# OpenGene/repaq

Hardware: AMD Instinct MI355X
Metric: raw FASTQ MB/s encode+decode (higher is better)
Workload: dtype u8; 1 GPU; configs[2]: synthetic NovaSeq PE150 two files (-i/-I), 2 x 4.01 GB FASTQ (fqgen profile 1, 11200000 pairs, seed 3, N 20 ppm), -k 1000, encode + decode; chunks_per_gpu=3360, parity=unchecked (checked with --full)

## Files before the change

### repaq_amd/csrc/enc/gather_tiles.h

```cpp
#pragma once
#define G2_CAP 23552u
#define G2_SE_OK 1
#define G2_CNT 256u
struct __attribute__((packed, aligned(1))) GU16g { uint32_t a, b, c, d; };
__device__ __forceinline__ void pack4_codes(uint32_t w, uint32_t& code, uint32_t& nb, uint32_t& bad) {
    const uint32_t idx = (w >> 1) & 0x03030303u;
    const uint32_t ok = eq_bytes_full(__builtin_amdgcn_perm(0u, 0x47544341u, idx), w);
    code = ((__builtin_amdgcn_perm(0u, 0x00020301u, idx) & ok) * 0x01041040u) >> 24;
    nb = 0; bad = 0;
    if (ok != 0xFFFFFFFFu) { const uint32_t isn = eq_bytes_full(w, 0x4E4E4E4Eu); nb = ((isn & 0x01010101u) * 0x01020408u) >> 24;
            bad = (((~ok & ~isn) & 0x01010101u) * 0x01020408u) >> 24; }
}
__device__ __forceinline__ void pack4_codes_rc(uint32_t w, uint32_t& code, uint32_t& nb) {
    const uint32_t u = w & 0xDFDFDFDFu, idx = (u >> 1) & 0x03030303u;
    const uint32_t ok = eq_bytes_full(__builtin_amdgcn_perm(0u, 0x47544341u, idx), u);
    code = ((__builtin_amdgcn_perm(0u, 0x03010002u, idx) & ok) * 0x01041040u) >> 24;
    nb = ((~ok & 0x01010101u) * 0x01020408u) >> 24;
}
__device__ __forceinline__ bool pack16_fast(const uint32_t (&w)[4], uint32_t& code) {
    uint32_t diff = 0; code = 0;
#pragma unroll
    for (int i = 0; i < 4; i++) {
        const uint32_t idx = (w[i] >> 1) & 0x03030303u;
        diff |= __builtin_amdgcn_perm(0u, 0x47544341u, idx) ^ w[i];
        code |= ((__builtin_amdgcn_perm(0u, 0x00020301u, idx) * 0x01041040u) >> 24) << (8 * i);
    }
    return diff == 0;
}
__device__ __forceinline__ uint32_t g2_rev2x16(uint32_t v) {
    v = bswap32(v); v = ((v >> 4) & 0x0F0F0F0Fu) | ((v & 0x0F0F0F0Fu) << 4); return ((v >> 2) & 0x33333333u) | ((v & 0x33333333u) << 2);
}
struct G2Geo { uint32_t a00, a01, end0, end1, base1; };
struct G2Read { bool on, rc; uint32_t len, qsrc, ssrc, qpos, ld, gi; };
struct G2Bound { uint32_t l0, l1, q; };
struct G2MRaw { uint4 lo4; uint32_t pg; };
#ifdef RFQ_SIMT_EMULATION
__device__ __forceinline__ uint32_t ld_uniform(const uint32_t* p) { return *p; }
#else
__device__ __forceinline__ uint32_t ld_uniform(const uint32_t* p) { return *(const __attribute__((address_space(4))) uint32_t*)(uintptr_t)p; }
#endif
__device__ __forceinline__ G2Bound g2_bound(const Text& T, bool two, const uint32_t* __restrict__ pq, uint32_t r) {
    G2Bound b;
    if (two) { const size_t k = 4 * (size_t)(r >> 1); b.l0 = ld_uniform(T.lo[0] + k); b.l1 = ld_uniform(T.lo[1] + k); }
    else { b.l0 = ld_uniform(T.lo[0] + 4 * (size_t)r); b.l1 = 0u; }
    b.q = ld_uniform(pq + r);
    return b;
}
__device__ __forceinline__ G2Geo g2_geo(const G2Bound& b, const G2Bound& e, bool two) {
    G2Geo g; g.a00 = b.l0 & ~15u; g.end0 = e.l0; g.a01 = two ? b.l1 & ~15u : 0u; g.end1 = two ? e.l1 : 0u;
    g.base1 = two ? (((g.end0 - g.a00 + 15u) & ~15u) + 16u) : 0u;
    return g;
}
__device__ __forceinline__ void g2_stage1(const uint8_t* __restrict__ fq, uint32_t n, uint32_t a0, uint32_t end, uint4* l4, uint32_t tid) {
    const uint32_t nb = end - a0, ng = (nb + 15u) / 16u;
    const uint8_t* src = fq + a0;
    const uint32_t nfull = (uint64_t)a0 + 16ull * ng <= (uint64_t)n ? ng : ng - 1u;
    for (uint32_t i = tid; i < nfull; i += blockDim.x)
        __builtin_amdgcn_global_load_lds((const __attribute__((address_space(1))) void*)(src + 16 * (size_t)i),
                (__attribute__((address_space(3))) void*)(l4 + (i - (tid & 63u))), 16, 0, 0);
    if (nfull < ng && tid == 0) { uint8_t* const bytes = (uint8_t*)l4;
            for (uint32_t k = 0; k < 16; k++) bytes[16 * nfull + k] = a0 + 16 * nfull + k < n ? src[16 * (size_t)nfull + k] : (uint8_t)0xFF; }
}
__device__ __forceinline__ void g2_stage(const Text& T, bool two, const G2Geo& g, uint4* buf4, uint32_t tid) {
    g2_stage1(T.fq[0], T.n[0], g.a00, g.end0, buf4, tid);
    if (two) g2_stage1(T.fq[1], T.n[1], g.a01, g.end1, buf4 + g.base1 / 16, tid);
}
__device__ __forceinline__ G2MRaw g2_mraw(const Text& T, const uint32_t* __restrict__ pq, uint32_t cur, uint32_t j, uint32_t cnt) {
    G2MRaw r; r.lo4 = make_uint4(0, 0, 0, 0); r.pg = 0;
    if (j < cnt) { const uint32_t gi = cur + j; int s_; uint32_t r_; read_loc(T, gi, s_, r_); r.lo4 = *(const uint4*)(t_lo(T, s_) + 4 * (size_t)r_); r.pg = pq[gi]; }
    return r;
}
__device__ __forceinline__ G2Read g2_read(const Text& T, const G2MRaw& r, const G2Geo& g, uint32_t f, uint32_t pq0, bool il, uint32_t cur, uint32_t j, uint32_t cnt) {
    G2Read m; m.on = j < cnt; m.rc = false; m.len = m.qsrc = m.ssrc = m.qpos = m.ld = 0; m.gi = cur + j;
    if (m.on) {
        const uint32_t gi = cur + j; int s_; uint32_t r_; read_loc(T, gi, s_, r_);
        const uint32_t lb = s_ ? g.base1 : 0u, a = s_ ? g.a01 : g.a00;
        m.len = r.lo4.z - 1u - r.lo4.y; m.ssrc = lb + (r.lo4.y - a); m.qsrc = lb + (r.lo4.w - a);
        m.qpos = r.pg - pq0; m.ld = (r.pg >> 4) + gi;
        m.rc = il && ((gi - f) & 1u);
    }
    return m;
}
__device__ __forceinline__ void g2_bases(const uint8_t* s_text, const G2Read& m, uint32_t part, uint32_t P, uint32_t* __restrict__ lpk, uint16_t* __restrict__ lnb,
        uint8_t* __restrict__ rflag, uint8_t* __restrict__ rn) {
    const uint32_t ng = (m.len + 15u) >> 4;
    for (uint32_t gi = part; gi < ng; gi += P) {
        uint32_t w[4], code = 0, nbits = 0;
        const uint32_t nv0 = m.len - 16u * gi;
        const bool tail = nv0 < 16u && m.len >= 16u; const uint32_t tsh = tail ? 16u - nv0 : 0u;
        auto blank = [&](uint32_t from, uint32_t to) { for (uint32_t k = from; k < to; k++) { uint32_t& x = w[k >> 2]; const uint32_t sh = 8u * (k & 3u);
                x = (x & ~(0xFFu << sh)) | (0x41u << sh); } };
        if (!m.rc) {
            lds_get16(s_text, m.ssrc + (tail ? m.len - 16u : 16u * gi), w);
            if (nv0 < 16u && !tail) blank(nv0, 16u);
            if (!pack16_fast(w, code)) {
                uint32_t bad = 0; code = 0;
#pragma unroll
                for (int i = 0; i < 4; i++) { uint32_t c4, n4, b4; pack4_codes(w[i], c4, n4, b4); code |= c4 << (8 * i); nbits |= n4 << (4 * i); bad |= b4 << (4 * i); }
                if (bad) rflag[m.gi] = 1;
            }
        } else {
            lds_get16(s_text, tail ? m.ssrc : m.ssrc + m.len - 16u * gi - 16u, w);
            if (nv0 < 16u && !tail) blank(0u, 16u - nv0);
            if (pack16_fast(w, code)) code = ~g2_rev2x16(code);
            else {
                const uint32_t x0 = bswap32(w[3]), x1 = bswap32(w[2]), x2 = bswap32(w[1]), x3 = bswap32(w[0]); w[0] = x0; w[1] = x1; w[2] = x2; w[3] = x3; code = 0;
#pragma unroll
                for (int i = 0; i < 4; i++) { uint32_t c4, n4; pack4_codes_rc(w[i], c4, n4); code |= c4 << (8 * i); nbits |= n4 << (4 * i); }
            }
        }
        code >>= 2u * tsh; nbits >>= tsh;
        if (nv0 < 16u) { code &= (1u << (2u * nv0)) - 1u; nbits &= (1u << nv0) - 1u; }
        lpk[m.ld + gi] = code; lnb[m.ld + gi] = (uint16_t)nbits;
        if (nbits) rn[m.gi] = 1;
    }
}
__device__ __forceinline__ void g2_compose(const uint8_t* s_text, const G2Read& m, uint32_t part, uint32_t P, uint8_t* qd, uint32_t* __restrict__ lpk,
        uint16_t* __restrict__ lnb, uint8_t* __restrict__ rflag, uint8_t* __restrict__ rn, QualCount& qc) {
    if (!m.on) return;
    {
        const uint32_t n = m.len; uint8_t* const o = qd + m.qpos; const bool rc = m.rc;
        if (n >= 16u) {
            const uint32_t ng = (n + 15u) >> 4;
            for (uint32_t gi = part; gi < ng; gi += P) {
                uint32_t p0 = 16u * gi, dup = 0; if (p0 + 16u > n) { dup = p0 + 16u - n; p0 = n - 16u; }
                uint32_t w[4]; lds_get16(s_text, rc ? m.qsrc + n - p0 - 16u : m.qsrc + p0, w);
                if (rc) { const uint32_t x0 = bswap32(w[3]), x1 = bswap32(w[2]), x2 = bswap32(w[1]), x3 = bswap32(w[0]); w[0] = x0; w[1] = x1; w[2] = x2; w[3] = x3; }
                { GU16g v; v.a = w[0]; v.b = w[1]; v.c = w[2]; v.d = w[3]; *(GU16g*)(o + p0) = v; }
                if (!dup) qc.group(m.qpos + p0, w[0], w[1], w[2], w[3]);
                else for (uint32_t k = dup; k < 16u; k++) qc(m.qpos + p0 + k, (uint8_t)(w[k >> 2] >> (8u * (k & 3u))));
            }
        } else for (uint32_t i = part; i < n; i += P) { const uint8_t q = s_text[rc ? m.qsrc + n - 1u - i : m.qsrc + i]; o[i] = q; qc(m.qpos + i, q); }
    }
    g2_bases(s_text, m, part, P, lpk, lnb, rflag, rn);
}
#define G2_REFN 256u
#define G2_REFS 128u
struct G2Ref { uint32_t nl, n1l, n2o, len, stl, lane, tile, nb, tb; int s; };
struct G2Acc { uint32_t bits, fail; };
__device__ __forceinline__ bool lane_bytes_eq(const uint8_t* tx, uint32_t a, uint32_t b, uint32_t n, bool on) {
    bool eq = true;
    for (uint32_t o = 0; __any(on && eq && o < n); o += 16u) {
        if (on && eq && o < n) {
            uint32_t p0 = o, v = n - o; if (v < 16u && n >= 16u) { p0 = n - 16u; v = 16u; }
            uint32_t x[4], y[4]; lds_get16(tx, a + p0, x); lds_get16(tx, b + p0, y);
            unsigned long long dl = (((unsigned long long)(x[1] ^ y[1])) << 32) | (x[0] ^ y[0]), dh = (((unsigned long long)(x[3] ^ y[3])) << 32) | (x[2] ^ y[2]);
            if (v < 16u) { dl &= v >= 8u ? ~0ull : (1ull << (8u * v)) - 1ull; dh &= v > 8u ? (1ull << (8u * (v - 8u))) - 1ull : 0ull; }
            if (dl | dh) eq = false;
        }
    }
    return eq;
}
__device__ __forceinline__ bool lane_bytes_eq32(const uint8_t* tx, uint32_t a, uint32_t b, uint32_t n) {
    uint32_t x[4], y[4]; lds_get16(tx, a, x); lds_get16(tx, b, y);
    unsigned long long dl = (((unsigned long long)(x[1] ^ y[1])) << 32) | (x[0] ^ y[0]), dh = (((unsigned long long)(x[3] ^ y[3])) << 32) | (x[2] ^ y[2]);
    if (n < 16u) { dl &= n >= 8u ? ~0ull : (1ull << (8u * n)) - 1ull; dh &= n > 8u ? (1ull << (8u * (n - 8u))) - 1ull : 0ull; }
    else { const uint32_t t = n - 16u; lds_get16(tx, a + t, x); lds_get16(tx, b + t, y); dl |= (((unsigned long long)(x[1] ^ y[1])) << 32) | (x[0] ^ y[0]);
            dh |= (((unsigned long long)(x[3] ^ y[3])) << 32) | (x[2] ^ y[2]); }
    return (dl | dh) == 0ull;
}
__device__ __forceinline__ bool g2_eq_ref(const uint8_t* tx, uint32_t a, uint32_t ro, uint32_t cap, const uint8_t* g0, uint32_t off0, uint32_t len0, uint32_t n,
        bool on) {
    const bool slow = on && len0 > cap, big = on && !slow && n > 32u; bool eq = true;
    if (on && !slow && !big && n) eq = lane_bytes_eq32(tx, a, ro + off0, n);
    if (__any(big)) { if (!lane_bytes_eq(tx, a, ro + off0, n, big)) eq = false; }
    if (slow) for (uint32_t i = 0; i < n && eq; i++) if (tx[a + i] != g0[off0 + i]) eq = false;
    return eq;
}
__device__ __forceinline__ uint32_t g2_atoi(const uint8_t* tx, uint32_t a, uint32_t n) {
    if (n == 0) return 0u;
    const unsigned long long w = lds_get8(tx, a); const uint32_t c0 = (uint32_t)w & 0xFFu;
    if (n > 8u || c0 == ' ' || (c0 >= 9u && c0 <= 13u) || c0 == '+' || c0 == '-') return (uint32_t)dev_atoi(tx + a, n);
    const unsigned long long x = w ^ 0x3030303030303030ull;
    const unsigned long long nd = (((x & 0x7F7F7F7F7F7F7F7Full) + 0x7676767676767676ull) | x) & 0x8080808080808080ull;
    uint32_t m = nd ? (uint32_t)(__ffsll((long long)nd) - 1) >> 3 : 8u; if (m > n) m = n;
    if (m == 0) return 0u;
    const unsigned long long X = x << (8u * (8u - m));
    const uint32_t hi4 = (uint32_t)X, lo4 = (uint32_t)(X >> 32);
    const uint32_t uh = ((hi4 << 3) + (hi4 << 1) + (hi4 >> 8)) & 0x00FF00FFu, ul = ((lo4 << 3) + (lo4 << 1) + (lo4 >> 8)) & 0x00FF00FFu;
    const uint32_t vh = mul24(uh & 0xFFu, 100u) + (uh >> 16), vl = mul24(ul & 0xFFu, 100u) + (ul >> 16);
    return mul24(vh, 10000u) + vl;
}
__device__ __forceinline__ uint32_t ctz64_or64(unsigned long long m) { return m ? (uint32_t)(__ffsll((long long)m) - 1) : 64u; }
__device__ __forceinline__ void g2_parse(const Text& T, const ReadTab& R, const uint8_t* tx, uint32_t refn, uint32_t refs, const G2Geo& g, const G2Ref& r0, uint32_t f,
        uint32_t cur, uint32_t cnt,
                                         bool can0, uint32_t dpos, uint32_t dch, G2Acc& acc) {
    const uint32_t l = (uint32_t)lane_id(); const bool on = l < cnt; const uint32_t gi = cur + l;
    uint32_t nsrc = 0, nl = 0, sl = 0, tsrc = 0, tl = 0;
    if (on) {
        int s_; uint32_t r_; read_loc(T, gi, s_, r_);
        const uint4 lo4 = *(const uint4*)(t_lo(T, s_) + 4 * (size_t)r_);
        const uint32_t lb = s_ ? g.base1 : 0u, a = s_ ? g.a01 : g.a00;
        nsrc = lb + (lo4.x - a); nl = lo4.y - 1u - lo4.x; sl = lo4.z - 1u - lo4.y; tsrc = lb + (lo4.z - a); tl = lo4.w - 1u - lo4.z;
    }
    unsigned long long Cm = 0, Sm = 0;
    {
        uint32_t c[4], sp_[4];
#pragma unroll
        for (int p = 0; p < 4; p++) { uint32_t w[4]; lds_get16(tx, nsrc + 16u * (uint32_t)p, w); const uint4 q = make_uint4(w[0], w[1], w[2], w[3]);
                c[p] = eq_mask16c(q, 0x3A3A3A3Au); sp_[p] = eq_mask16c(q, 0x20202020u); }
        const unsigned long long keep = !on ? 0ull : (nl >= 64u ? ~0ull : (1ull << nl) - 1ull);
        Cm = ((((unsigned long long)(c[2] | (c[3] << 16))) << 32) | (c[0] | (c[1] << 16))) & keep;
        Sm = ((((unsigned long long)(sp_[2] | (sp_[3] << 16))) << 32) | (sp_[0] | (sp_[1] << 16))) & keep;
    }
    const uint32_t sp = ctz64_or64(Sm);
    unsigned long long cb = sp < 64u ? Cm & ((1ull << sp) - 1ull) : Cm;
    const uint32_t k = (uint32_t)__popcll(cb);
    uint32_t cpos[8];
#pragma unroll
    for (int i = 1; i <= 7; i++) { cpos[i] = ctz64_or64(cb); cb &= cb - 1ull; }
    const bool at7 = cpos[7] < 64u, at_sp = !at7 && sp < 64u;
    const bool undecided = on && !at7 && !at_sp && nl > 64u;
    uint32_t ok = 0, n1l = nl, n2o = nl, lane_v = 0, tile_v = 0, x_v = 0, y_v = 0;
    if (on && (at7 || (at_sp && k >= 4u))) {
        ok = 1; n2o = at7 ? cpos[7] : sp;
        const bool k4 = at_sp && k == 4u, k5 = at_sp && k == 5u;
        n1l = k4 ? cpos[4] : cpos[3];
        const uint32_t ls = (k4 ? cpos[4] : cpos[3]) + 1u, le = k4 ? sp : cpos[4];
        lane_v = g2_atoi(tx, nsrc + ls, le - ls) & 0xFFu;
        if (k >= 5u) { const uint32_t ts = (k5 ? cpos[5] : cpos[4]) + 1u, te = k5 ? sp : cpos[5]; tile_v = g2_atoi(tx, nsrc + ts, te - ts) & 0xFFFFu; }
        if (k >= 6u) x_v = g2_atoi(tx, nsrc + cpos[5] + 1u, cpos[6] - cpos[5] - 1u);
        if (at7) y_v = g2_atoi(tx, nsrc + cpos[6] + 1u, cpos[7] - cpos[6] - 1u);
        else if (k == 6u) y_v = g2_atoi(tx, nsrc + cpos[6] + 1u, sp - cpos[6] - 1u);
    }
    if (__any(undecided)) {
        if (undecided) { const Meta m = dev_parse_name(tx + nsrc, nl); ok = m.ok; n1l = m.name1_len; n2o = m.name2_off; lane_v = m.lane; tile_v = m.tile; x_v = m.x;
                y_v = m.y; }
    }
    if (on) { R.name1_len[gi] = n1l; R.name2_off[gi] = n2o; R.x[gi] = x_v; R.y[gi] = y_v; R.tile[gi] = (uint16_t)tile_v; R.lane[gi] = (uint8_t)lane_v;
            R.ok[gi] = (uint8_t)ok; }
    const uint32_t n2l = nl - n2o, n2l0 = r0.nl - r0.n2o;
    const uint8_t* g0n = t_fq(T, r0.s) + r0.nb; const uint8_t* g0s = t_fq(T, r0.s) + r0.tb;
    const bool st_eq = g2_eq_ref(tx, tsrc, refs, G2_REFS, g0s, 0u, r0.stl, tl, on && tl == r0.stl);
    const bool n1_eq = g2_eq_ref(tx, nsrc, refn, G2_REFN, g0n, 0u, r0.nl, n1l, on && n1l == r0.n1l);
    const bool n2_eq = g2_eq_ref(tx, nsrc + n2o, refn, G2_REFN, g0n, r0.n2o, r0.nl, n2l, on && n2l == n2l0);
    const uint32_t pn = wave_shr1(nsrc, 0u), pnl = wave_shr1(nl, 0u), pn2o = wave_shr1(n2o, 0u), plane = wave_shr1(lane_v, 0u), ptile = wave_shr1(tile_v,
            0u), px = wave_shr1(x_v, 0u), py = wave_shr1(y_v, 0u);
    const uint32_t rel = gi - f; const bool odd = on && can0 && (rel & 1u);
    bool fa = false;
    if (__any(odd)) {
        const uint32_t pn2l = pnl - pn2o; const bool same_len = odd && pn2l == n2l;
        if (odd && !same_len) fa = true;
        const uint32_t ma = pn + pn2o, mb = nsrc + n2o; const bool small = same_len && n2l <= 16u, big = same_len && !small;
        if (small && n2l) {
            uint32_t x[4], y[4]; lds_get16(tx, ma, x); lds_get16(tx, mb, y);
            if (dch != 0u && dpos < n2l) {
                const uint32_t sh = 8u * (dpos & 3u);
#pragma unroll
                for (int q = 0; q < 4; q++) if ((dpos >> 2) == (uint32_t)q) x[q] = (x[q] & ~(0xFFu << sh)) | (dch << sh);
            }
            unsigned long long dl = (((unsigned long long)(x[1] ^ y[1])) << 32) | (x[0] ^ y[0]), dh = (((unsigned long long)(x[3] ^ y[3])) << 32) | (x[2] ^ y[2]);
            if (n2l < 16u) { dl &= n2l >= 8u ? ~0ull : (1ull << (8u * n2l)) - 1ull; dh &= n2l > 8u ? (1ull << (8u * (n2l - 8u))) - 1ull : 0ull; }
            if (dl | dh) fa = true;
        }
        if (__any(big)) {
            if (!lane_bytes_eq(tx, ma, mb, dpos < n2l ? dpos : n2l, big)) fa = true;
            if (big && dpos < n2l) { if ((dch != 0u ? dch : (uint32_t)tx[ma + dpos]) != (uint32_t)tx[mb + dpos]) fa = true; }
            if (!lane_bytes_eq(tx, ma + dpos + 1u, mb + dpos + 1u, n2l > dpos + 1u ? n2l - dpos - 1u : 0u, big && dpos + 1u < n2l)) fa = true;
        }
    }
    if (on) {
        uint32_t b = 0;
        if (sl == r0.len) b |= 1u << 0;
        if (n1l == r0.n1l) b |= 1u << 1;
        if (n2l == n2l0) b |= 1u << 2;
        if (tl == r0.stl) b |= 1u << 3;
        if (tl == r0.stl && st_eq) b |= 1u << 4;
        if (lane_v == r0.lane) b |= 1u << 5;
        if (tile_v == r0.tile) b |= 1u << 6;
        if (n1l == r0.n1l && n1_eq) b |= 1u << 7;
        const bool e2 = n2l == n2l0 && n2_eq;
        if (e2) b |= 1u << 8;
        if (e2 || (rel & 1u)) b |= 1u << 9;
        acc.bits &= b;
        R.eq2[gi] = e2 ? 1 : 0;
        if (odd) {
            const bool fb = plane != lane_v || ptile != tile_v || px != x_v || py != y_v;
            if (fa || fb) { const uint32_t key = (rel << 1) | (fa ? 0u : 1u); if (key < acc.fail) acc.fail = key; }
        }
    }
}
__device__ __forceinline__ void g2_mirror_ends(const Text& T, const uint8_t* tx, const G2Geo& g, uint32_t cur, uint32_t cnt, uint32_t* mirror_err) {
    const uint32_t l = (uint32_t)lane_id(); bool bad = false;
    if (l < cnt) {
        int s_; uint32_t r_; read_loc(T, cur + l, s_, r_);
        if (s_ == 1) {
            const uint32_t* const p = t_lo(T, 1) + 4 * (size_t)r_; const uint32_t o = g.base1 - g.a01, n = T.n[1];
            const uint32_t e1 = p[1], e2 = p[2], e3 = p[3], e4 = p[4];
            bad = tx[o + e1 - 1u] != '\n' || tx[o + e2 - 1u] != '\n' || tx[o + e3 - 1u] != '\n' || (e4 - 1u < n && tx[o + e4 - 1u] != '\n');
        }
    }
    if (__any(bad)) { if (l == 0u) atomicOr(mirror_err, (uint32_t)DE_MIRROR_FAIL); }
}
#define G2_PLANES 5u
#define G2_PLANE_EXC 4u
#define G2_RARE_LIST 255u
struct G2Planes { uint32_t* planes; uint64_t pstride; uint32_t pw, nd; uint32_t* rare; uint32_t* mirror_err; };
__device__ __forceinline__ uint32_t ctl_flags4(uint32_t w) { return (w - 0x10101010u) & ~w & 0x80808080u; }
__device__ __forceinline__ uint32_t ctl_count16(const uint4& q) {
    return (uint32_t)__popc(ctl_flags4(q.x)) + (uint32_t)__popc(ctl_flags4(q.y)) + (uint32_t)__popc(ctl_flags4(q.z)) + (uint32_t)__popc(ctl_flags4(q.w));
}
__device__ __forceinline__ uint32_t g2_ctl_count(const uint4* l4, uint32_t head, uint32_t nb, uint32_t tid) {
    const uint32_t ng = (nb + 15u) >> 4; uint32_t c = 0;
    for (uint32_t i0 = 0; i0 < ng; i0 += 256u) { const uint32_t i = i0 + tid; if (i < ng) c += ctl_count16(l4[i]); }
    if (tid < 32u) {
        const uint32_t k = tid & 15u, p = tid < 16u ? k : nb + k;
        if (tid < 16u ? k < head : p < 16u * ng) c -= ((const uint8_t*)l4)[p] < 0x10u ? 1u : 0u;
    }
    return c;
}
__device__ __forceinline__ void g2_rare_or(uint32_t* __restrict__ gpl, uint64_t pstride, uint32_t* __restrict__ rare_c, uint32_t plane, uint32_t pos) {
    const uint32_t old = atomicOr(&gpl[(size_t)plane * pstride + (pos >> 5)], 1u << (pos & 31u));
    if (old == 0u) { const uint32_t k = atomicAdd(rare_c, 1u); if (k < G2_RARE_LIST) rare_c[1u + k] = (plane << 28) | (pos >> 5); }
}
__device__ __forceinline__ void g2_quals_masks(const uint8_t* tx, const G2Read& m, uint32_t part, uint32_t P, uint32_t* pl, uint32_t pw, uint32_t wbase, uint32_t nd,
                                               uint32_t pat0, uint32_t pat1, uint32_t pat2, uint32_t patm, const DevHeader* __restrict__ D, uint8_t* qd, uint32_t* __restrict__ gpl, uint64_t pstride,
                                               uint32_t* __restrict__ segm_c, int* __restrict__ segc_c, uint32_t n_seg, uint32_t* __restrict__ rare_c) {
    if (!m.on) return;
    const uint32_t n = m.len, ng = (n + 15u) >> 4; const bool rc = m.rc;
    for (uint32_t gi = part; gi < ng; gi += P) {
        const uint32_t p0 = 16u * gi, nv = n - p0;
        uint32_t w[4]; lds_get16(tx, rc ? m.qsrc + n - p0 - 16u : m.qsrc + p0, w);
        if (rc) { const uint32_t x0 = bswap32(w[3]), x1 = bswap32(w[2]), x2 = bswap32(w[1]), x3 = bswap32(w[0]); w[0] = x0; w[1] = x1; w[2] = x2; w[3] = x3; }
        const uint32_t valid = nv >= 16u ? 0xFFFFu : (1u << nv) - 1u;
        const uint4 q = make_uint4(w[0], w[1], w[2], w[3]);
        const uint32_t bit = m.qpos + p0 - wbase, wi = bit >> 5, sh = bit & 31u;
        uint32_t known = eq_mask16c(q, patm);
        auto plane = [&](uint32_t d, uint32_t pat) {
            const uint32_t mv = eq_mask16c(q, pat); known |= mv;
            const unsigned long long x = (unsigned long long)(mv & valid) << sh;
            if ((uint32_t)x) atomicOr(&pl[d * pw + wi], (uint32_t)x);
            if ((uint32_t)(x >> 32)) atomicOr(&pl[d * pw + wi + 1u], (uint32_t)(x >> 32));
        };
        if (nd > 0u) plane(0u, pat0);
        if (nd > 1u) plane(1u, pat1);
        if (nd > 2u) plane(2u, pat2);
        uint32_t rest = ~known & valid;
        while (rest) {
            const uint32_t k = (uint32_t)__ffs((int)rest) - 1u; rest &= rest - 1u;
            const uint32_t ww = k < 8u ? (k < 4u ? w[0] : w[1]) : (k < 12u ? w[2] : w[3]), pos = m.qpos + p0 + k, b = (ww >> (8u * (k & 3u))) & 0xFFu;
            const uint32_t j = D->stream_of[b];
            if (j < 4u && j < D->n_normal) { const size_t si = (size_t)j * n_seg + pos / PC_SEG_POS; g2_rare_or(gpl, pstride, rare_c, j, pos); atomicAdd(&segm_c[si], 1u);
                    atomicMax(&segc_c[si], (int)pos); }
            else { qd[pos] = (uint8_t)b; g2_rare_or(gpl, pstride, rare_c, G2_PLANE_EXC, pos); atomicAdd(&segm_c[(size_t)EXC_SLOT * n_seg + pos / PC_SEG_POS], 1u); }
        }
    }
}
__device__ __forceinline__ void g2_flush_masks(uint32_t* pl, uint32_t pw, uint32_t nd, uint32_t dense3 , uint32_t* s_carry, uint32_t* __restrict__ gpl, uint64_t pstride,
                                               uint32_t gw0, uint32_t nw, bool carry, bool or_first, bool or_last,
                                               size_t seg_index0 , uint32_t n_seg, uint32_t* __restrict__ segm, int* __restrict__ segc) {
    const uint32_t tid = threadIdx.x, seg0 = (gw0 << 5) / PC_SEG_POS;
    for (uint32_t d = 0; d < nd; d++) {
        const uint32_t v = (dense3 >> (8u * d)) & 0xFFu;
        uint32_t c01 = 0; int l0 = -1, l1 = -1;
        for (uint32_t i = tid; i < nw; i += blockDim.x) {
            const uint32_t x = pl[d * pw + i]; pl[d * pw + i] = 0u;
            const bool last = i + 1u == nw;
            if (last && carry) { s_carry[d] = x; continue; }
            const uint32_t gw = gw0 + i; uint32_t* const dst = gpl + (size_t)v * pstride + gw;
            if ((i == 0u && or_first) || (last && or_last)) { if (x) atomicOr(dst, x); } else *dst = x;
            if (x) { const uint32_t sg = ((gw << 5) / PC_SEG_POS) - seg0; const int lp = (int)((gw << 5) + 31u - (uint32_t)__clz((int)x));
                     c01 += (uint32_t)__popc(x) << (16u * sg); if (sg) { if (lp > l1) l1 = lp; } else if (lp > l0) l0 = lp; }
        }
        if (!carry && tid == 0) s_carry[d] = 0u;
        c01 = wave_sum(c01); l0 = wave_max(l0); l1 = wave_max(l1);
        if ((tid & 63u) == 0 && c01) {
            const size_t si = seg_index0 + (size_t)v * n_seg + seg0;
            if (c01 & 0xFFFFu) { atomicAdd(&segm[si], c01 & 0xFFFFu); atomicMax(&segc[si], l0); }
            if ((c01 >> 16) && seg0 + 1u < n_seg) { atomicAdd(&segm[si + 1u], c01 >> 16); atomicMax(&segc[si + 1u], l1); }
        }
    }
}
__global__ void k_mask_bounds(const uint32_t* __restrict__ pq, const uint32_t* __restrict__ first, const uint64_t* __restrict__ qbase, uint32_t* __restrict__ planes,
        uint64_t pstride, const DevHeader* __restrict__ D, uint32_t nd, uint32_t bx,
                              const uint32_t* __restrict__ only) {
    const uint32_t c = blockIdx.x; if (only && !only[c]) return;
    const uint32_t f = first[c], e = first[c + 1], pq0 = pq[f];
    uint32_t per = ((e - f) + bx - 1) / bx; per = (per + 1u) & ~1u;
    for (uint32_t b = 1u + threadIdx.x; b < bx; b += blockDim.x) {
        const uint32_t gs = f + b * per; if (gs >= e) break;
        const uint32_t w = (uint32_t)(qbase[c] >> 5) + ((pq[gs] - pq0) >> 5);
        for (uint32_t d = 0; d < nd; d++) planes[(size_t)D->dense[d] * pstride + w] = 0u;
    }
}
template <bool MASKS, int PAIRED = -1> __global__ void __launch_bounds__(256, 6) k_gather2(Text T_, ReadTab R, const uint32_t* __restrict__ first, const uint64_t* __restrict__ qbase,
                                                 const DevHeader* __restrict__ D, uint8_t* __restrict__ qcat, uint32_t* __restrict__ lpk, uint16_t* __restrict__ lnb, uint8_t* __restrict__ rflag,
                                                 uint8_t* __restrict__ rn, uint32_t* __restrict__ segm, int* __restrict__ segc, uint32_t n_seg, uint32_t kshift,
                                                 uint32_t* __restrict__ cbits, uint32_t* __restrict__ cfail, const uint32_t* __restrict__ only, uint32_t text4, G2Planes M) {
    Text T = T_; if (PAIRED >= 0) T.paired = PAIRED;
    constexpr bool PE = PAIRED != 0;
    RFQ_DYN_SHARED(uint4, g2_lds);
    __shared__ uint32_t sh[MASKS ? 1 : G2_CNT]; __shared__ int sh_last[MASKS ? 1 : G2_CNT]; __shared__ uint8_t s_slot[MASKS ? 16 : 256];
            __shared__ uint32_t s_r0[8], s_carry[4], s_mctl;
    const uint32_t REFN = (text4 - 1u) * 16u, REFS = REFN + G2_REFN + 16u;
    uint32_t* const pl = (uint32_t*)(g2_lds + text4 + (G2_REFN + G2_REFS + 32u) / 16u);
    const uint32_t c = blockIdx.y;
    const bool redo = only != nullptr;
    if (redo && !only[c]) return;
    const uint32_t tid = threadIdx.x;
    const uint32_t* __restrict__ pq = R.pq;
    const uint32_t nn_s = D->n_normal < NPOS_SLOT ? D->n_normal : NPOS_SLOT, nslot = nn_s + 1u;
    uint32_t nrep = 1;
    if (!MASKS) {
        for (uint32_t i = tid; i < G2_CNT; i += blockDim.x) { sh[i] = 0; sh_last[i] = -1; }
        while (nrep < 16u && 4u * nrep * nslot <= G2_CNT) nrep *= 2u;
        for (uint32_t i = tid; i < 256; i += blockDim.x) { const uint32_t j = D->stream_of[i]; s_slot[i] = (uint8_t)(j < nn_s ? j : nn_s); }
    } else {
        for (uint32_t i = tid; i < M.nd * M.pw; i += blockDim.x) pl[i] = 0u;
        if (tid < 4u) s_carry[tid] = 0u;
    }
    if (tid == 0) s_mctl = 0u;
    const uint32_t f = first[c], e = first[c + 1];
    const bool two = PE && T.paired == 1, can0 = PE && T.paired != 0 && D->support_interleaved != 0, il = can0 && !redo;
    const uint32_t dpos = D->name2_diff_pos, dch = D->name2_diff_char;
    uint8_t* const qd = qcat + qbase[c]; const uint32_t pq0 = pq[f];
    uint32_t per = ((e - f) + gridDim.x - 1) / gridDim.x; per = (per + 1u) & ~1u;
    const uint32_t gs = f + blockIdx.x * per, ge = gs + per < e ? gs + per : e;
    const uint32_t K = 1u << kshift, pshift = 8u - kshift, P = 1u << pshift;
    const uint32_t jj = tid >> pshift, j = ((jj << 1) & (K - 1u)) | (jj >> (kshift - 1u)), part = tid & (P - 1u);
    QualCount qc; qc.cnt = sh; qc.last = sh_last; qc.slot = s_slot; qc.major = D->major & 0xFFu; qc.seg0 = 0; qc.nslot = nslot; qc.rep = tid & (nrep - 1u);
            qc.hot_ok = D->stream_of[D->major & 0xFFu] == 0xFF;
    const uint32_t nd = MASKS ? M.nd : 0u, dense3 = (uint32_t)D->dense[0] | ((uint32_t)D->dense[1] << 8) | ((uint32_t)D->dense[2] << 16);
    const uint32_t pat0 = (uint32_t)D->normal[dense3 & 0xFFu] * 0x01010101u, pat1 = (uint32_t)D->normal[(dense3 >> 8) & 0xFFu] * 0x01010101u, pat2 = (uint32_t)D->normal[(dense3 >> 16) & 0xFFu] * 0x01010101u, patm = (D->major & 0xFFu) * 0x01010101u;
    uint32_t* const gpl = M.planes + (MASKS ? (size_t)(qbase[c] >> 5) : (size_t)0);
    uint4* const buf4 = g2_lds + 1; const uint8_t* const tx = (const uint8_t*)buf4;
    G2Ref r0 = {}; G2Acc acc; acc.bits = CF_ALL; acc.fail = 0xFFFFFFFFu;
    const bool parse = !redo && gs < ge;
    const bool mirror = (PAIRED == 1 || (PAIRED == -1 && !MASKS)) && two && !redo && M.mirror_err != nullptr;
    uint32_t mwant = 0;
    if (parse) {
        uint32_t r_; read_loc(T, f, r0.s, r_); const uint32_t* p = t_lo(T, r0.s) + 4 * (size_t)r_;
        const uint32_t p0 = p[0], p1 = p[1], p2 = p[2], p3 = p[3];
        r0.nb = p0; r0.nl = p1 - 1u - p0; r0.len = p2 - 1u - p1; r0.tb = p2; r0.stl = p3 - 1u - p2;
        uint8_t* const wr = (uint8_t*)buf4;
        if (tid < r0.nl) wr[REFN + tid] = t_fq(T, r0.s)[r0.nb + tid];
        if (tid < G2_REFS && tid < r0.stl) wr[REFS + tid] = t_fq(T, r0.s)[r0.tb + tid];
        __syncthreads();
        if (tid == 0) {
            const Meta m0 = r0.nl <= G2_REFN ? dev_parse_name(tx + REFN, r0.nl) : dev_parse_name(t_fq(T, r0.s) + r0.nb, r0.nl);
            s_r0[0] = m0.name1_len; s_r0[1] = m0.name2_off; s_r0[2] = m0.lane; s_r0[3] = m0.tile;
        }
    }
    __syncthreads();
    if (parse) { r0.n1l = s_r0[0]; r0.n2o = s_r0[1]; r0.lane = s_r0[2]; r0.tile = s_r0[3]; }
    uint32_t tix = blockIdx.x + blockIdx.y;
    const uint32_t ntile = gs < ge ? (ge - gs + K - 1u) >> kshift : 0u;
    auto tile_at = [&](uint32_t t_) -> uint32_t { const uint32_t x = gs + (t_ << kshift); return x < ge ? x : ge; };
    G2Bound b0 = g2_bound(T, two, pq, tile_at(0)), b1 = g2_bound(T, two, pq, tile_at(1)), b2 = g2_bound(T, two, pq, tile_at(2));
    G2MRaw mr = g2_mraw(T, pq, gs, j, ntile ? tile_at(1) - gs : 0u);
    if (ntile) g2_stage(T, two, g2_geo(b0, b1, two), buf4, tid);
    for (uint32_t t = 0; t < ntile; t++, tix++) {
        const uint32_t cur = tile_at(t), cnt = tile_at(t + 1u) - cur;
        const G2Geo g = g2_geo(b0, b1, two);
        const G2Read m = g2_read(T, mr, g, f, pq0, il, cur, j, cnt);
        const uint32_t qbeg = b0.q - pq0, qend = b1.q - pq0;
        { const uint32_t ncur = tile_at(t + 1u); mr = g2_mraw(T, pq, ncur, j, tile_at(t + 2u) - ncur); }
        const G2Bound b3 = g2_bound(T, two, pq, tile_at(t + 3u));
        __syncthreads();
        qc.seg0 = qbeg / PC_SEG_POS;
        if (parse && (uint32_t)wave_id() == (tix & 3u)) { g2_parse(T, R, tx, REFN, REFS, g, r0, f, cur, cnt, can0, dpos, dch, acc);
                if (mirror) g2_mirror_ends(T, tx, g, cur, cnt, M.mirror_err); }
        if (MASKS) {
            if (tid < nd && s_carry[tid]) atomicOr(&pl[tid * M.pw], s_carry[tid]);
            g2_quals_masks(tx, m, part, P, pl, M.pw, qbeg & ~31u, nd, pat0, pat1, pat2, patm, D, qd, gpl, M.pstride, segm + (size_t)c * MAX_STREAMS * n_seg,
                    segc + (size_t)c * MAX_STREAMS * n_seg, n_seg, M.rare + (size_t)c * (1u + G2_RARE_LIST));
            g2_bases(tx, m, part, P, lpk, lnb, rflag, rn);
        } else g2_compose(tx, m, part, P, qd, lpk, lnb, rflag, rn, qc);
        if (mirror) {
            const uint32_t end1 = g.end1 < T.n[1] ? g.end1 : T.n[1];
            const uint32_t mctl = wave_sum(g2_ctl_count(buf4 + g.base1 / 16u, b0.l1 - g.a01, end1 - g.a01, tid));
            if ((tid & 63u) == 0 && mctl) atomicAdd(&s_mctl, mctl);
            mwant += 2u * cnt - (g.end1 > T.n[1] ? 1u : 0u);
        }
        __syncthreads();
        if (t + 1u < ntile) g2_stage(T, two, g2_geo(b1, b2, two), buf4, tid);
        if (MASKS) {
            const uint32_t gw0 = qbeg >> 5, nw = ((qend + 31u) >> 5) - gw0; const bool last_tile = cur + cnt >= ge;
            g2_flush_masks(pl, M.pw, nd, dense3, s_carry, gpl, M.pstride, gw0, nw, !last_tile && (qend & 31u) != 0u, cur == gs && gs > f && (qbeg & 31u) != 0u,
                    last_tile && ge < e && (qend & 31u) != 0u,
                           (size_t)c * MAX_STREAMS * n_seg, n_seg, segm, segc);
        } else qual_flush(sh, sh_last, nrep, nslot, qc.seg0, c, nn_s, segm, segc, n_seg);
        b0 = b1; b1 = b2; b2 = b3;
    }
    if (parse) {
        const uint32_t bits = wave_and(acc.bits), fail = wave_min(acc.fail);
        if ((tid & 63u) == 0) { if (bits != CF_ALL) atomicAnd(&cbits[c], bits); if (fail != 0xFFFFFFFFu) atomicMin(&cfail[c], fail); }
    }
    if (mirror) {
        __syncthreads();
        if (tid == 0 && s_mctl != mwant) atomicOr(M.mirror_err, (uint32_t)DE_MIRROR_FAIL);
    }
}
__device__ __forceinline__ uint32_t dense_mask_of(const DevHeader* __restrict__ D, uint32_t nd) { uint32_t m = 0;
        for (uint32_t d = 0; d < nd; d++) m |= 1u << D->dense[d]; return m; }
__device__ __forceinline__ void k_rare_zero_chunk(uint32_t* __restrict__ planes, uint64_t pstride, uint32_t dense_mask, const uint32_t* __restrict__ pq,
        const uint32_t* __restrict__ first, const uint64_t* __restrict__ qbase, uint32_t c) {
    const uint32_t nw = (pq[first[c + 1]] - pq[first[c]] + 31u) >> 5; const size_t w0 = (size_t)(qbase[c] >> 5);
    for (uint32_t v = 0; v < G2_PLANES; v++) if (!((dense_mask >> v) & 1u)) for (uint32_t i = threadIdx.x; i < nw; i += blockDim.x) planes[(size_t)v * pstride + w0 + i] = 0u;
}
__global__ void k_gather_redo_reset(const uint32_t* __restrict__ only, uint32_t* __restrict__ segm, int* __restrict__ segc, uint32_t n_seg,
                                    uint32_t* __restrict__ xplane, uint64_t pstride, const DevHeader* __restrict__ D, uint32_t nd, const uint32_t* __restrict__ pq, const uint32_t* __restrict__ first, const uint64_t* __restrict__ qbase) {
    const uint32_t c = blockIdx.x; if (!only[c]) return;
    const size_t k = (size_t)c * MAX_STREAMS * n_seg;
    for (uint32_t i = threadIdx.x; i < MAX_STREAMS * n_seg; i += blockDim.x) { segm[k + i] = 0u; segc[k + i] = -1; }
    if (xplane) { k_rare_zero_chunk(xplane, pstride, dense_mask_of(D, nd), pq, first, qbase, c);
            if (threadIdx.x == 0) xplane[(size_t)G2_PLANES * pstride + (size_t)c * (1u + G2_RARE_LIST)] = 0u; }
}
__global__ void k_rare_cleanup(uint32_t* __restrict__ rare, uint32_t* __restrict__ planes, uint64_t pstride, const DevHeader* __restrict__ D, uint32_t nd,
        const uint32_t* __restrict__ pq, const uint32_t* __restrict__ first, const uint64_t* __restrict__ qbase) {
    const uint32_t c = blockIdx.x; uint32_t* const rc = rare + (size_t)c * (1u + G2_RARE_LIST); const uint32_t n = rc[0]; if (!n) return;
    if (n <= G2_RARE_LIST) { const size_t w0 = (size_t)(qbase[c] >> 5); for (uint32_t i = threadIdx.x; i < n; i += blockDim.x) { const uint32_t e = rc[1u + i];
            planes[(size_t)(e >> 28) * pstride + w0 + (e & 0x0FFFFFFFu)] = 0u; } }
    else k_rare_zero_chunk(planes, pstride, dense_mask_of(D, nd), pq, first, qbase, c);
    __syncthreads();
    if (threadIdx.x == 0) rc[0] = 0u;
}
__device__ __forceinline__ uint32_t loose_codes(const uint32_t* __restrict__ lpk, uint32_t ld, uint32_t b) {
    const uint32_t d = ld + (b >> 4), sh = 2u * (b & 15u); const uint32_t lo = lpk[d];
    return sh ? (uint32_t)(((((unsigned long long)lpk[d + 1]) << 32) | lo) >> sh) : lo;
}
__device__ __forceinline__ uint32_t loose_nbits(const uint16_t* __restrict__ lnb, uint32_t ld, uint32_t b) {
    const uint32_t d = ld + (b >> 4), sh = b & 15u; const uint32_t lo = lnb[d];
    return (sh ? ((((uint32_t)lnb[d + 1]) << 16) | lo) >> sh : lo) & 0xFFFFu;
}
#define SP_OWN 4096u
#define SP_EXTRA 8u
#define SP_U 3
struct __attribute__((packed, aligned(4))) SpU8 { uint32_t a, b; };
struct __attribute__((packed, aligned(2))) SpU4 { uint32_t a; };
__global__ void __launch_bounds__(256) k_seqpack(const uint32_t* __restrict__ pq, const uint32_t* __restrict__ sd, const U4* __restrict__ ptot,
        const uint32_t* __restrict__ first, const uint32_t* __restrict__ ilv, const int8_t* __restrict__ ovb,
                                                 const DevHeader* __restrict__ D, const uint64_t* __restrict__ sbase, const uint32_t* __restrict__ lpk, const uint16_t* __restrict__ lnb, const uint8_t* __restrict__ rn,
                                                 uint32_t* __restrict__ spk, uint16_t* __restrict__ snm, uint32_t* __restrict__ ncount, uint32_t* __restrict__ nmap, uint32_t* __restrict__ segm, int* __restrict__ segc, uint32_t n_seg,
                                                 uint32_t rshift) {
    __shared__ uint32_t s_sd[256 + SP_EXTRA + 1], s_ld[256 + SP_EXTRA], s_sk[256 + SP_EXTRA]; __shared__ uint8_t s_own[SP_OWN];
    __shared__ uint8_t s_hn[256 + SP_EXTRA + 8];
    const uint32_t c = blockIdx.y, f = first[c], e = first[c + 1], tid = threadIdx.x;
    const uint32_t ps0 = sd[f], S = ptot[c].d;
    const bool il = ilv[c] != 0, enc = il && (D->flags & H_PE_OVERLAP); const int shift = D->overlap_shift;
    uint32_t* const ok = spk + (size_t)(sbase[c] >> 4); uint16_t* const on = snm + (size_t)(sbase[c] >> 4);
    const uint32_t nshift = nmap_shift(S); uint32_t* const nm = nmap + (size_t)c * NMAP_WORDS;
    const size_t nsi = ((size_t)c * MAX_STREAMS + NPOS_SLOT) * n_seg;
    uint32_t nsum = 0;
    auto skip_of = [&](uint32_t g) -> uint32_t {
        if (enc && ((g - f) & 1u)) { const int ov = (int)ovb[g >> 1] - shift; if (ov > 0) return (uint32_t)ov; }
        return 0u;
    };
    const uint32_t R = 1u << rshift;
    for (uint32_t r0 = f + blockIdx.x * R; r0 < e; r0 += gridDim.x * R) {
        const uint32_t nr = e - r0 < R ? e - r0 : R, nx = e - r0 < R + SP_EXTRA ? e - r0 : R + SP_EXTRA;
        for (uint32_t t = tid; t <= nx; t += blockDim.x) {
            const uint32_t g = r0 + t; s_sd[t] = g < e ? sd[g] - ps0 : S;
            if (t < nx) { s_ld[t] = (pq[g] >> 4) + g; s_sk[t] = skip_of(g); s_hn[t] = rn[g]; } else s_hn[t] = 0;
        }
        __syncthreads();
        const uint32_t kbase = (s_sd[0] + 15u) >> 4, kend = (s_sd[nr] + 15u) >> 4;
        if (tid < nr) { const uint32_t ka = (s_sd[tid] + 15u) >> 4, kb = (s_sd[tid + 1] + 15u) >> 4; for (uint32_t k = ka; k < kb; k++) s_own[k - kbase] = (uint8_t)tid; }
        __syncthreads();
        const uint32_t ndw = kend - kbase;
        for (uint32_t i0 = 0; i0 < ndw; i0 += blockDim.x * SP_U) {
            struct Dw { uint32_t k, need, t1, jj, sh, sh2, take2, n, n2; unsigned long long c, c2; } q[SP_U]; uint32_t nres[SP_U];
#pragma unroll
            for (int u = 0; u < SP_U; u++) nres[u] = 0;
#pragma unroll
            for (int u = 0; u < SP_U; u++) {
                Dw& x = q[u]; x.need = 0; x.take2 = 0; x.k = x.t1 = x.jj = x.sh = x.sh2 = x.n = x.n2 = 0; x.c = x.c2 = 0;
                const uint32_t i = i0 + (uint32_t)u * blockDim.x + tid;
                if (i < ndw) {
                    const uint32_t k = kbase + i, j = s_own[i];
                    const uint32_t B = 16u * k, si = B - s_sd[j], need = S - B < 16u ? S - B : 16u, av = s_sd[j + 1] - B, t1 = need < av ? need : av;
                    const uint32_t b0 = s_sk[j] + si, d = s_ld[j] + (b0 >> 4);
                    x.k = k; x.need = need; x.t1 = t1; x.sh = b0 & 15u; x.jj = j + 1u;
                    { const SpU8 v = *(const SpU8*)(lpk + d); x.c = (((unsigned long long)v.b) << 32) | v.a; x.n = s_hn[j] ? ((const SpU4*)(lnb + d))->a : 0u; }
// ... 104 lines not shown
```

Baseline: 1.139 million MB/s.

## Fold mirror control-byte check into per-read parse and pack paths

Replaces the separate per-tile pass that counted control bytes over the whole file-1 staged text with checks spread into existing read-processing paths. The quality, base and parse routines now test for control bytes inline and flag a mirror failure on a hit, which drops the extra LDS sweep, the wave reduction, the shared counter and the final block barrier. Inline checks are compiled in through a CHK template flag. The trade is extra per-read branching and LDS reads in the parse wave, plus a subtly different validation rule that could miss or add detections.

```diff
diff --git a/repaq_amd/csrc/enc/gather_tiles.h b/repaq_amd/csrc/enc/gather_tiles.h
--- a/repaq_amd/csrc/enc/gather_tiles.h
+++ b/repaq_amd/csrc/enc/gather_tiles.h
@@ -81,8 +81,18 @@
     }
     return m;
 }
-__device__ __forceinline__ void g2_bases(const uint8_t* s_text, const G2Read& m, uint32_t part, uint32_t P, uint32_t* __restrict__ lpk, uint16_t* __restrict__ lnb,
-        uint8_t* __restrict__ rflag, uint8_t* __restrict__ rn) {
+__device__ __forceinline__ uint32_t ctl_flags4(uint32_t w) { return (w - 0x10101010u) & ~w & 0x80808080u; }
+__device__ __forceinline__ uint32_t ctl_mask16(const uint4& q) {
+    const uint32_t lo = udot4(ctl_flags4(q.y), 0x80402010u, udot4(ctl_flags4(q.x), 0x08040201u, 0u));
+    const uint32_t hi = udot4(ctl_flags4(q.w), 0x80402010u, udot4(ctl_flags4(q.z), 0x08040201u, 0u));
+    return ((hi << 8) | lo) >> 7;
+}
+__device__ __forceinline__ void g2_mirror_fail(uint32_t* mirror_err) { atomicOr(mirror_err, (uint32_t)DE_MIRROR_FAIL); }
+__device__ __forceinline__ uint32_t ctl_any16(const uint32_t (&w)[4]) {
+    return (((w[0] - 0x10101010u) & ~w[0]) | ((w[1] - 0x10101010u) & ~w[1]) | ((w[2] - 0x10101010u) & ~w[2]) | ((w[3] - 0x10101010u) & ~w[3])) & 0x80808080u;
+}
+template <bool CHK> __device__ __forceinline__ void g2_bases(const uint8_t* s_text, const G2Read& m, uint32_t part, uint32_t P, uint32_t* __restrict__ lpk, uint16_t* __restrict__ lnb,
+        uint8_t* __restrict__ rflag, uint8_t* __restrict__ rn, bool mirror, uint32_t* mirror_err) {
     const uint32_t ng = (m.len + 15u) >> 4;
     for (uint32_t gi = part; gi < ng; gi += P) {
         uint32_t w[4], code = 0, nbits = 0;
@@ -97,7 +107,7 @@
                 uint32_t bad = 0; code = 0;
 #pragma unroll
                 for (int i = 0; i < 4; i++) { uint32_t c4, n4, b4; pack4_codes(w[i], c4, n4, b4); code |= c4 << (8 * i); nbits |= n4 << (4 * i); bad |= b4 << (4 * i); }
-                if (bad) rflag[m.gi] = 1;
+                if (bad) { rflag[m.gi] = 1; if (CHK && mirror && (m.gi & 1u) && ctl_any16(w)) g2_mirror_fail(mirror_err); }
             }
         } else {
             lds_get16(s_text, tail ? m.ssrc : m.ssrc + m.len - 16u * gi - 16u, w);
@@ -107,6 +117,7 @@
                 const uint32_t x0 = bswap32(w[3]), x1 = bswap32(w[2]), x2 = bswap32(w[1]), x3 = bswap32(w[0]); w[0] = x0; w[1] = x1; w[2] = x2; w[3] = x3; code = 0;
 #pragma unroll
                 for (int i = 0; i < 4; i++) { uint32_t c4, n4; pack4_codes_rc(w[i], c4, n4); code |= c4 << (8 * i); nbits |= n4 << (4 * i); }
+                if (CHK && mirror && (m.gi & 1u) && nbits && ctl_any16(w)) g2_mirror_fail(mirror_err);
             }
         }
         code >>= 2u * tsh; nbits >>= tsh;
@@ -115,8 +126,8 @@
         if (nbits) rn[m.gi] = 1;
     }
 }
-__device__ __forceinline__ void g2_compose(const uint8_t* s_text, const G2Read& m, uint32_t part, uint32_t P, uint8_t* qd, uint32_t* __restrict__ lpk,
-        uint16_t* __restrict__ lnb, uint8_t* __restrict__ rflag, uint8_t* __restrict__ rn, QualCount& qc) {
+template <bool CHK> __device__ __forceinline__ void g2_compose(const uint8_t* s_text, const G2Read& m, uint32_t part, uint32_t P, uint8_t* qd, uint32_t* __restrict__ lpk,
+        uint16_t* __restrict__ lnb, uint8_t* __restrict__ rflag, uint8_t* __restrict__ rn, QualCount& qc, bool mirror, uint32_t* mirror_err) {
     if (!m.on) return;
     {
         const uint32_t n = m.len; uint8_t* const o = qd + m.qpos; const bool rc = m.rc;
@@ -125,14 +136,16 @@
             for (uint32_t gi = part; gi < ng; gi += P) {
                 uint32_t p0 = 16u * gi, dup = 0; if (p0 + 16u > n) { dup = p0 + 16u - n; p0 = n - 16u; }
                 uint32_t w[4]; lds_get16(s_text, rc ? m.qsrc + n - p0 - 16u : m.qsrc + p0, w);
+                if (CHK && mirror && (m.gi & 1u) && ctl_any16(w)) g2_mirror_fail(mirror_err);
                 if (rc) { const uint32_t x0 = bswap32(w[3]), x1 = bswap32(w[2]), x2 = bswap32(w[1]), x3 = bswap32(w[0]); w[0] = x0; w[1] = x1; w[2] = x2; w[3] = x3; }
                 { GU16g v; v.a = w[0]; v.b = w[1]; v.c = w[2]; v.d = w[3]; *(GU16g*)(o + p0) = v; }
                 if (!dup) qc.group(m.qpos + p0, w[0], w[1], w[2], w[3]);
                 else for (uint32_t k = dup; k < 16u; k++) qc(m.qpos + p0 + k, (uint8_t)(w[k >> 2] >> (8u * (k & 3u))));
             }
-        } else for (uint32_t i = part; i < n; i += P) { const uint8_t q = s_text[rc ? m.qsrc + n - 1u - i : m.qsrc + i]; o[i] = q; qc(m.qpos + i, q); }
-    }
-    g2_bases(s_text, m, part, P, lpk, lnb, rflag, rn);
+        } else for (uint32_t i = part; i < n; i += P) { const uint8_t q = s_text[rc ? m.qsrc + n - 1u - i : m.qsrc + i]; o[i] = q; qc(m.qpos + i, q);
+                if (CHK && mirror && (m.gi & 1u) && q < 0x10u) g2_mirror_fail(mirror_err); }
+    }
+    g2_bases<CHK>(s_text, m, part, P, lpk, lnb, rflag, rn, mirror, mirror_err);
 }
 #define G2_REFN 256u
 #define G2_REFS 128u
@@ -181,27 +194,53 @@
     const uint32_t vh = mul24(uh & 0xFFu, 100u) + (uh >> 16), vl = mul24(ul & 0xFFu, 100u) + (ul >> 16);
     return mul24(vh, 10000u) + vl;
 }
+__device__ __forceinline__ bool lane_ctl(const uint8_t* tx, uint32_t a, uint32_t n, bool on) {
+    bool hit = false;
+    for (uint32_t o = 0; __any(on && o < n); o += 16u) {
+        if (on && o < n) {
+            uint32_t p0 = o, v = n - o; if (v < 16u && n >= 16u) { p0 = n - 16u; v = 16u; }
+            uint32_t x[4]; lds_get16(tx, a + p0, x);
+            uint32_t mk = ctl_mask16(make_uint4(x[0], x[1], x[2], x[3])); if (v < 16u) mk &= (1u << v) - 1u;
+            if (mk) hit = true;
+        }
+    }
+    return hit;
+}
 __device__ __forceinline__ uint32_t ctz64_or64(unsigned long long m) { return m ? (uint32_t)(__ffsll((long long)m) - 1) : 64u; }
-__device__ __forceinline__ void g2_parse(const Text& T, const ReadTab& R, const uint8_t* tx, uint32_t refn, uint32_t refs, const G2Geo& g, const G2Ref& r0, uint32_t f,
+template <bool CHK> __device__ __forceinline__ void g2_parse(const Text& T, const ReadTab& R, const uint8_t* tx, uint32_t refn, uint32_t refs, const G2Geo& g, const G2Ref& r0, uint32_t f,
         uint32_t cur, uint32_t cnt,
-                                         bool can0, uint32_t dpos, uint32_t dch, G2Acc& acc) {
+                                         bool can0, uint32_t dpos, uint32_t dch, G2Acc& acc, bool mirror, uint32_t* mirror_err) {
     const uint32_t l = (uint32_t)lane_id(); const bool on = l < cnt; const uint32_t gi = cur + l;
     uint32_t nsrc = 0, nl = 0, sl = 0, tsrc = 0, tl = 0;
+    bool s1 = false, mbad = false;
     if (on) {
         int s_; uint32_t r_; read_loc(T, gi, s_, r_);
         const uint4 lo4 = *(const uint4*)(t_lo(T, s_) + 4 * (size_t)r_);
         const uint32_t lb = s_ ? g.base1 : 0u, a = s_ ? g.a01 : g.a00;
         nsrc = lb + (lo4.x - a); nl = lo4.y - 1u - lo4.x; sl = lo4.z - 1u - lo4.y; tsrc = lb + (lo4.z - a); tl = lo4.w - 1u - lo4.z;
+        if (CHK && mirror && s_ == 1) {
+            const uint32_t e4 = t_lo(T, 1)[4 * (size_t)r_ + 4], ql = e4 - 1u - lo4.w, qsrc = lb + (lo4.w - a);
+            s1 = true;
+            mbad = tx[nsrc + nl] != '\n' || tx[tsrc - 1u] != '\n' || tx[tsrc + tl] != '\n' || (e4 - 1u < T.n[1] && tx[qsrc + ql] != '\n') || ql != sl;
+            if (tl == 1u && tx[tsrc] < 0x10u) mbad = true;
+        }
     }
     unsigned long long Cm = 0, Sm = 0;
     {
         uint32_t c[4], sp_[4];
 #pragma unroll
         for (int p = 0; p < 4; p++) { uint32_t w[4]; lds_get16(tx, nsrc + 16u * (uint32_t)p, w); const uint4 q = make_uint4(w[0], w[1], w[2], w[3]);
-                c[p] = eq_mask16c(q, 0x3A3A3A3Au); sp_[p] = eq_mask16c(q, 0x20202020u); }
+                c[p] = eq_mask16c(q, 0x3A3A3A3Au); sp_[p] = eq_mask16c(q, 0x20202020u);
+                if (CHK && mirror) { const uint32_t nv = nl > 16u * (uint32_t)p ? nl - 16u * (uint32_t)p : 0u; if (s1 && (ctl_mask16(q) & (nv >= 16u ? 0xFFFFu : (1u << nv) - 1u))) mbad = true; } }
         const unsigned long long keep = !on ? 0ull : (nl >= 64u ? ~0ull : (1ull << nl) - 1ull);
         Cm = ((((unsigned long long)(c[2] | (c[3] << 16))) << 32) | (c[0] | (c[1] << 16))) & keep;
         Sm = ((((unsigned long long)(sp_[2] | (sp_[3] << 16))) << 32) | (sp_[0] | (sp_[1] << 16))) & keep;
+    }
+    if (CHK && mirror) {
+        const bool nlong = s1 && nl > 64u, tlong = s1 && tl != 1u;
+        if (__any(nlong)) { if (lane_ctl(tx, nsrc + 64u, nl - 64u, nlong)) mbad = true; }
+        if (__any(tlong)) { if (lane_ctl(tx, tsrc, tl, tlong)) mbad = true; }
+        if (__any(mbad)) { if (l == 0u) atomicOr(mirror_err, (uint32_t)DE_MIRROR_FAIL); }
     }
     const uint32_t sp = ctz64_or64(Sm);
     unsigned long long cb = sp < 64u ? Cm & ((1ull << sp) - 1ull) : Cm;
@@ -280,42 +319,17 @@
         }
     }
 }
-__device__ __forceinline__ void g2_mirror_ends(const Text& T, const uint8_t* tx, const G2Geo& g, uint32_t cur, uint32_t cnt, uint32_t* mirror_err) {
-    const uint32_t l = (uint32_t)lane_id(); bool bad = false;
-    if (l < cnt) {
-        int s_; uint32_t r_; read_loc(T, cur + l, s_, r_);
-        if (s_ == 1) {
-            const uint32_t* const p = t_lo(T, 1) + 4 * (size_t)r_; const uint32_t o = g.base1 - g.a01, n = T.n[1];
-            const uint32_t e1 = p[1], e2 = p[2], e3 = p[3], e4 = p[4];
-            bad = tx[o + e1 - 1u] != '\n' || tx[o + e2 - 1u] != '\n' || tx[o + e3 - 1u] != '\n' || (e4 - 1u < n && tx[o + e4 - 1u] != '\n');
-        }
-    }
-    if (__any(bad)) { if (l == 0u) atomicOr(mirror_err, (uint32_t)DE_MIRROR_FAIL); }
-}
 #define G2_PLANES 5u
 #define G2_PLANE_EXC 4u
 #define G2_RARE_LIST 255u
 struct G2Planes { uint32_t* planes; uint64_t pstride; uint32_t pw, nd; uint32_t* rare; uint32_t* mirror_err; };
-__device__ __forceinline__ uint32_t ctl_flags4(uint32_t w) { return (w - 0x10101010u) & ~w & 0x80808080u; }
-__device__ __forceinline__ uint32_t ctl_count16(const uint4& q) {
-    return (uint32_t)__popc(ctl_flags4(q.x)) + (uint32_t)__popc(ctl_flags4(q.y)) + (uint32_t)__popc(ctl_flags4(q.z)) + (uint32_t)__popc(ctl_flags4(q.w));
-}
-__device__ __forceinline__ uint32_t g2_ctl_count(const uint4* l4, uint32_t head, uint32_t nb, uint32_t tid) {
-    const uint32_t ng = (nb + 15u) >> 4; uint32_t c = 0;
-    for (uint32_t i0 = 0; i0 < ng; i0 += 256u) { const uint32_t i = i0 + tid; if (i < ng) c += ctl_count16(l4[i]); }
-    if (tid < 32u) {
-        const uint32_t k = tid & 15u, p = tid < 16u ? k : nb + k;
-        if (tid < 16u ? k < head : p < 16u * ng) c -= ((const uint8_t*)l4)[p] < 0x10u ? 1u : 0u;
-    }
-    return c;
-}
 __device__ __forceinline__ void g2_rare_or(uint32_t* __restrict__ gpl, uint64_t pstride, uint32_t* __restrict__ rare_c, uint32_t plane, uint32_t pos) {
     const uint32_t old = atomicOr(&gpl[(size_t)plane * pstride + (pos >> 5)], 1u << (pos & 31u));
     if (old == 0u) { const uint32_t k = atomicAdd(rare_c, 1u); if (k < G2_RARE_LIST) rare_c[1u + k] = (plane << 28) | (pos >> 5); }
 }
-__device__ __forceinline__ void g2_quals_masks(const uint8_t* tx, const G2Read& m, uint32_t part, uint32_t P, uint32_t* pl, uint32_t pw, uint32_t wbase, uint32_t nd,
+template <bool CHK> __device__ __forceinline__ void g2_quals_masks(const uint8_t* tx, const G2Read& m, uint32_t part, uint32_t P, uint32_t* pl, uint32_t pw, uint32_t wbase, uint32_t nd,
                                                uint32_t pat0, uint32_t pat1, uint32_t pat2, uint32_t patm, const DevHeader* __restrict__ D, uint8_t* qd, uint32_t* __restrict__ gpl, uint64_t pstride,
-                                               uint32_t* __restrict__ segm_c, int* __restrict__ segc_c, uint32_t n_seg, uint32_t* __restrict__ rare_c) {
+                                               uint32_t* __restrict__ segm_c, int* __restrict__ segc_c, uint32_t n_seg, uint32_t* __restrict__ rare_c, bool mirror, uint32_t* mirror_err) {
     if (!m.on) return;
     const uint32_t n = m.len, ng = (n + 15u) >> 4; const bool rc = m.rc;
     for (uint32_t gi = part; gi < ng; gi += P) {
@@ -340,6 +354,7 @@
             const uint32_t k = (uint32_t)__ffs((int)rest) - 1u; rest &= rest - 1u;
             const uint32_t ww = k < 8u ? (k < 4u ? w[0] : w[1]) : (k < 12u ? w[2] : w[3]), pos = m.qpos + p0 + k, b = (ww >> (8u * (k & 3u))) & 0xFFu;
             const uint32_t j = D->stream_of[b];
+            if (CHK && mirror && (m.gi & 1u) && b < 0x10u) g2_mirror_fail(mirror_err);
             if (j < 4u && j < D->n_normal) { const size_t si = (size_t)j * n_seg + pos / PC_SEG_POS; g2_rare_or(gpl, pstride, rare_c, j, pos); atomicAdd(&segm_c[si], 1u);
                     atomicMax(&segc_c[si], (int)pos); }
             else { qd[pos] = (uint8_t)b; g2_rare_or(gpl, pstride, rare_c, G2_PLANE_EXC, pos); atomicAdd(&segm_c[(size_t)EXC_SLOT * n_seg + pos / PC_SEG_POS], 1u); }
@@ -391,7 +406,7 @@
     constexpr bool PE = PAIRED != 0;
     RFQ_DYN_SHARED(uint4, g2_lds);
     __shared__ uint32_t sh[MASKS ? 1 : G2_CNT]; __shared__ int sh_last[MASKS ? 1 : G2_CNT]; __shared__ uint8_t s_slot[MASKS ? 16 : 256];
-            __shared__ uint32_t s_r0[8], s_carry[4], s_mctl;
+            __shared__ uint32_t s_r0[8], s_carry[4];
     const uint32_t REFN = (text4 - 1u) * 16u, REFS = REFN + G2_REFN + 16u;
     uint32_t* const pl = (uint32_t*)(g2_lds + text4 + (G2_REFN + G2_REFS + 32u) / 16u);
     const uint32_t c = blockIdx.y;
@@ -409,7 +424,6 @@
         for (uint32_t i = tid; i < M.nd * M.pw; i += blockDim.x) pl[i] = 0u;
         if (tid < 4u) s_carry[tid] = 0u;
     }
-    if (tid == 0) s_mctl = 0u;
     const uint32_t f = first[c], e = first[c + 1];
     const bool two = PE && T.paired == 1, can0 = PE && T.paired != 0 && D->support_interleaved != 0, il = can0 && !redo;
     const uint32_t dpos = D->name2_diff_pos, dch = D->name2_diff_char;
@@ -426,8 +440,9 @@
     uint4* const buf4 = g2_lds + 1; const uint8_t* const tx = (const uint8_t*)buf4;
     G2Ref r0 = {}; G2Acc acc; acc.bits = CF_ALL; acc.fail = 0xFFFFFFFFu;
     const bool parse = !redo && gs < ge;
-    const bool mirror = (PAIRED == 1 || (PAIRED == -1 && !MASKS)) && two && !redo && M.mirror_err != nullptr;
-    uint32_t mwant = 0;
+    constexpr bool CHK = PAIRED == 1 || (PAIRED == -1 && !MASKS);
+    const bool mirror = CHK && two && !redo && M.mirror_err != nullptr;
+    if (MASKS && mirror && ((tid == 0 && (D->major & 0xFFu) < 0x10u) || (tid < D->n_normal && D->normal[tid] < 0x10u))) atomicOr(M.mirror_err, (uint32_t)DE_MIRROR_FAIL);
     if (parse) {
         uint32_t r_; read_loc(T, f, r0.s, r_); const uint32_t* p = t_lo(T, r0.s) + 4 * (size_t)r_;
         const uint32_t p0 = p[0], p1 = p[1], p2 = p[2], p3 = p[3];
@@ -458,20 +473,13 @@
         const G2Bound b3 = g2_bound(T, two, pq, tile_at(t + 3u));
         __syncthreads();
         qc.seg0 = qbeg / PC_SEG_POS;
-        if (parse && (uint32_t)wave_id() == (tix & 3u)) { g2_parse(T, R, tx, REFN, REFS, g, r0, f, cur, cnt, can0, dpos, dch, acc);
-                if (mirror) g2_mirror_ends(T, tx, g, cur, cnt, M.mirror_err); }
+        if (parse && (uint32_t)wave_id() == (tix & 3u)) g2_parse<CHK>(T, R, tx, REFN, REFS, g, r0, f, cur, cnt, can0, dpos, dch, acc, mirror, M.mirror_err);
         if (MASKS) {
             if (tid < nd && s_carry[tid]) atomicOr(&pl[tid * M.pw], s_carry[tid]);
-            g2_quals_masks(tx, m, part, P, pl, M.pw, qbeg & ~31u, nd, pat0, pat1, pat2, patm, D, qd, gpl, M.pstride, segm + (size_t)c * MAX_STREAMS * n_seg,
-                    segc + (size_t)c * MAX_STREAMS * n_seg, n_seg, M.rare + (size_t)c * (1u + G2_RARE_LIST));
-            g2_bases(tx, m, part, P, lpk, lnb, rflag, rn);
-        } else g2_compose(tx, m, part, P, qd, lpk, lnb, rflag, rn, qc);
-        if (mirror) {
-            const uint32_t end1 = g.end1 < T.n[1] ? g.end1 : T.n[1];
-            const uint32_t mctl = wave_sum(g2_ctl_count(buf4 + g.base1 / 16u, b0.l1 - g.a01, end1 - g.a01, tid));
-            if ((tid & 63u) == 0 && mctl) atomicAdd(&s_mctl, mctl);
-            mwant += 2u * cnt - (g.end1 > T.n[1] ? 1u : 0u);
-        }
+            g2_quals_masks<CHK>(tx, m, part, P, pl, M.pw, qbeg & ~31u, nd, pat0, pat1, pat2, patm, D, qd, gpl, M.pstride, segm + (size_t)c * MAX_STREAMS * n_seg,
+                    segc + (size_t)c * MAX_STREAMS * n_seg, n_seg, M.rare + (size_t)c * (1u + G2_RARE_LIST), mirror, M.mirror_err);
+            g2_bases<CHK>(tx, m, part, P, lpk, lnb, rflag, rn, mirror, M.mirror_err);
+        } else g2_compose<CHK>(tx, m, part, P, qd, lpk, lnb, rflag, rn, qc, mirror, M.mirror_err);
         __syncthreads();
         if (t + 1u < ntile) g2_stage(T, two, g2_geo(b1, b2, two), buf4, tid);
         if (MASKS) {
@@ -485,10 +493,6 @@
     if (parse) {
         const uint32_t bits = wave_and(acc.bits), fail = wave_min(acc.fail);
         if ((tid & 63u) == 0) { if (bits != CF_ALL) atomicAnd(&cbits[c], bits); if (fail != 0xFFFFFFFFu) atomicMin(&cfail[c], fail); }
-    }
-    if (mirror) {
-        __syncthreads();
-        if (tid == 0 && s_mctl != mwant) atomicOr(M.mirror_err, (uint32_t)DE_MIRROR_FAIL);
     }
 }
 __device__ __forceinline__ uint32_t dense_mask_of(const DevHeader* __restrict__ D, uint32_t nd) { uint32_t m = 0;
```

Result: no change. 1.138 million MB/s (-0.1%).
